# DeepLearningZ/chanamq

Hardware: AMD Instinct MI355X
Metric: msgs/sec (whole node) + p50 publish→deliver latency, 1 KB payload, 1/2/4/8 GPUs (higher is better)
Workload: dtype uint8 (AMQP wire bytes; no floating-point compute)

## Files before the change

chanamq_amd/engine/dataplane.py:

```python

import ctypes
import time
from collections import defaultdict

import os

import numpy as np

from .. import ops
from ..protocol import constants as C
from .control import ControlError, ControlState
from .layout import (CONN_OUT, CONSUMED_REC, EGRESS_REF, RING_MOVE, CTRL_REC, CTRL_DGET, CTRL_TXBUF, INVALID, MF_HAS_TS,
                     MF_HOSTPUB, MF_PERSIST,
                     MF_ONEQ, MF_REDELIVERED, MF_RESTORE,
                     PERSIST_HDR, RDESC, SEG_IN, SEG_OUT, SS_CTRL, US_ACKED, US_PENDING, US_REQUEUE, USLOT,
                     chan_hash, direct_key, exch_hash, fnv1a64, topic_pattern_row, topic_word_offsets)

ONES64 = np.uint64((1 << 64) - 1)


def parse_persist(raw):
    raw = np.frombuffer(raw, np.uint8) if isinstance(raw, (bytes, bytearray)) else raw
    hdrs, data_of, off = [], {}, 0
    while off + PERSIST_HDR.itemsize <= len(raw):
# ... 848 lines not shown
            self.eng.launch(p)
            self._pending = self._xprev = p
            return (p, len(segs), t0, self.eng.egress_slot(p))
        p = self.eng.submit(segs, int(payload_ptr), int(payload_len), now, self.step_no, now, self.worker)
        self.step_no += 1
        if self.world > 1:
            self._pending = p
            cnt = self.eng.send_counts(p)
            if cnt[-1]:
                raise RuntimeError("cross-rank send buffers overflowed (xfer_desc_max / xfer_bytes)")
            self._send_counts = cnt[:-1]
            if self.exchanger is not None:
                recv = self.exchanger.exchange(self._send_counts, self.xfer_send_desc(), self.xfer_send_pay(),
                                               self.xfer_recv_desc(), self.xfer_recv_pay())
                if self.lag:
                    self.set_import(recv)
                else:
                    self.submit_b(recv)
        return (p, len(segs), t0, self.eng.egress_slot(p))

    def prefetch(self, payload_ptr, payload_len):
        return bool(self.eng.prefetch(int(payload_ptr), int(payload_len)))

    def submit_lockstep(self, segs, payload_ptr, payload_len, now_ms=None):
        if not (self.world > 1 and self.native_xchg):
            raise RuntimeError("submit_lockstep: needs a sharded plane built with native_xchg=1")
        now = int(time.time() * 1000) if now_ms is None else int(now_ms)
        t0 = time.perf_counter()
        p = self.eng.submit(segs, int(payload_ptr), int(payload_len), now, self.step_no, now, self.worker)
        self.step_no += 1
        q = self._xprev
        if q is not None:
            rc, _ = self.eng.exchange(q, 0)
            if rc != 0:
                self.eng.drop_exchange(q)
                raise RuntimeError(f"rank {self.rank}: native exchange failed (rc {rc}: a peer did not answer)")
        self.eng.launch_b(p)
        self._xprev = p
        return (p, len(segs), t0, self.eng.egress_slot(p))

    def _exchange_parity(self, q):
        cnt = self.eng.send_counts(q)
        if cnt[-1]:
            raise RuntimeError("cross-rank send buffers overflowed (xfer_desc_max / xfer_bytes)")
        self._send_counts = cnt[:-1]
        recv = self.exchanger.exchange(self._send_counts, self._xs[q][0], self._xs[q][1],
# ... 119 lines not shown
```

csrc/kernels/dataplane.hip:

```cpp
#include "dp_state.h"
#include "dp_util.h"

DEV void apply_deltas(const DS& d, const u8* buf, u32 tid, u32 nt, DeltaRec* lrec) {
  const DeltaHead h = *(const DeltaHead*)buf;
  const DeltaRec* recs = (const DeltaRec*)(buf + sizeof(DeltaHead));
  const u32* dirty = (const u32*)(recs + h.nrec);
  const uint4* data = (const uint4*)((const u8*)dirty + ((4u * h.ndirty + 15u) & ~15u));
  for (u32 r = tid; r < h.nrec; r += nt) lrec[r] = recs[r];
  __syncthreads();
  for (u32 i = tid; i < h.nchunk; i += nt) {
    u32 lo = 0, hi = h.nrec;
    while (hi - lo > 1) {
      const u32 mid = (lo + hi) >> 1;
      if (lrec[mid].chunk0 <= i) lo = mid; else hi = mid;
    }
    const DeltaRec r = lrec[lo];
    const u32 off = (i - r.chunk0) * 16u;
    const u32 n = r.len - off < 16u ? r.len - off : 16u;
    const uint4 v = data[i];
    u8* dst = (u8*)(uintptr_t)(r.dst + off);
    const u32 w[4] = {v.x, v.y, v.z, v.w};
    if (((uintptr_t)dst & 3) == 0 && (n & 3) == 0) {
      for (u32 k = 0; k < n / 4; ++k) ((u32*)dst)[k] = w[k];
    } else {
      for (u32 k = 0; k < n; ++k) dst[k] = (u8)(w[k >> 2] >> (8 * (k & 3)));
    }
  }
  __syncthreads();
  for (u32 k = tid; k < h.ndirty; k += nt) {
    const u32 ch = dirty[k];
    if (atomicExch(&d.ch_dirty[ch], 1u) == 0) d.dirty_list[atomicAdd(d.n_dirty, 1u)] = ch;
  }
  __threadfence();
  __syncthreads();
}
__global__ __launch_bounds__(1024) void k_apply_deltas(DS d, const u8* buf) {
  __shared__ DeltaRec lrec[DELTA_REC_MAX];
  apply_deltas(d, buf, threadIdx.x, 1024, lrec);
}

__global__ __launch_bounds__(64) void k_h2d_wait(DS d) {
  const u64 sig = d.in->h2d_sig, sig2 = d.in->h2d_sig2;
  if (!sig) return;
  const u32 lim = d.in->h2d_polls ? d.in->h2d_polls : (1u << 24);
  if (threadIdx.x == 0)
    for (u32 it = 0; it < lim; ++it) {
      if (__hip_atomic_load((const i64*)sig, __ATOMIC_RELAXED, __HIP_MEMORY_SCOPE_SYSTEM) == 0 &&
          (!sig2 || __hip_atomic_load((const i64*)sig2, __ATOMIC_RELAXED, __HIP_MEMORY_SCOPE_SYSTEM) == 0))
        break;
      __builtin_amdgcn_s_sleep(4);
    }
  __syncthreads();
  __builtin_amdgcn_fence(__ATOMIC_ACQUIRE, "");
}

__global__ __launch_bounds__(1024) void k_stage(DS d) {
  __shared__ u32 lds[1024 / 64 + 1];
  __shared__ StepIn s_in;
  __shared__ DeltaRec lrec[DELTA_REC_MAX];
  const u32 tid = threadIdx.x;
  if (tid == 0) {
    s_in = *d.in_h;
    *d.in = s_in;
  }
  __syncthreads();
  if (s_in.delta_bytes) apply_deltas(d, d.delta_h, tid, 1024, lrec);
  const u32 nseg = s_in.nseg;
  {
    u32* c = (u32*)d.ctr;
    for (u32 k = tid; k < sizeof(Counters) / 4; k += 1024)
      if (k * 4 < offsetof(Counters, log_head)) c[k] = 0;
    if (tid == 0) {
      d.ctr->n_grow = 0; d.tot[TS_NMOVE] = 0; d.tot[TS_NDEFER] = 0; d.tot[TS_TTL_BUDGET] = 0;
      d.tot[TS_NDGET] = 0;
      d.tot[TS_SPILL_USED] = 0;
      d.tot[TS_HOP_N] = 0;
// ... 3480 lines not shown
```

csrc/kernels/dp_frame_scan.h:

```cpp
#pragma once
#include "dp_state.h"
#include "dp_util.h"

struct FInfo { u32 type, ch, size; bool complete, valid_hdr; };

DEV FInfo frame_at(const u8* b, u32 p, u32 L, u32 fmax) {
  FInfo f;
  f.complete = false;
  f.valid_hdr = false;
  f.type = 0; f.ch = 0; f.size = 0;
  if (p + 7 > L) return f;
  f.type = b[p];
  f.ch = be16(b + p + 1);
  f.size = be32(b + p + 3);
  bool tok = f.type == 1 || f.type == 2 || f.type == 3 || f.type == 8;
  bool sok = fmax == 0 || f.size + 8 <= fmax;
  f.valid_hdr = tok && sok;
  if (f.valid_hdr && (u64)p + 8 + f.size <= L) f.complete = (b[p + 7 + f.size] == 0xCE);
  return f;
}

DEV i32 chan_lookup(const DS& d, u32 conn, u32 ch) {
  const u32* m = d.chmap + (u64)conn * d.chmap_size;
  u32 mask = d.chmap_size - 1;
// ... 91 lines not shown
    const i32 v = d.x_hval[slot];
    if (v < 0) break;
    if (d.x_hkey[slot] == hk) { xs = v; break; }
  }
  if (xs < 0 || d.x_type[xs] != EX_DIRECT) return false;
  const u64 k = fnv1a64_dev(name, n) ^ (u64(xs) * 0x9E3779B97F4A7C15ULL);
  for (u32 j = 0; j <= d.dhash_mask; ++j) {
    const u32 s = (u32)(k + j) & d.dhash_mask;
    const i32 ex = d.d_exch[s];
    if (ex < 0) return false;
    if (ex == xs && d.d_key[s] == k && word_eq(d.kpool + d.d_kb_off[s], d.d_kb_len[s], name, n)) {
      if (d.d_q_n[s] != 1) return false;
      const u32 qq = d.d_q[d.d_q_off[s]];
      const u32 ex_owner = d.q_excl[qq];
      if (!d.q_active[qq] || d.q_owner[qq] != d.my_rank || (ex_owner && ex_owner != conn + 1)) return false;
      q = qq;
      noack = b[a + 1 + n] & 1u;
      return true;
    }
  }
  return false;
}

DEV void frame_scan_seg(const DS& d, const u32 s) {
  __shared__ uint4 fs_pool[FS_POOL / 16];
  __shared__ u32 sc[FS_NT / 64 + 1];
  __shared__ u32 sh_m, sh_over, sh_ok, sh_nf, sh_stop, sh_brk;
  __shared__ u32 sh_cmd_base, sh_frag_base, sh_ncmd;
  __shared__ u32 sh_get0, sh_gch, sh_gq, sh_gna, sh_gbase;
  __shared__ u32 sh_split;

  const u32 tid = threadIdx.x;
  const u32 conn = d.segs[s].conn;
  const u32 L = d.seg_total[s];
  const u32 seg_len = d.segs[s].len, seg_cl = L - seg_len, src = d.segs[s].src;
  const u64 ing_rel = (u64)d.in->ingress - (u64)d.work;
  const bool ing_ok = d.scan_inplace && d.world == 1 && (u64)d.in->ingress > (u64)d.work && ing_rel + src + L + 64 < (1ull << 32) &&
                      d.tot[TS_WORK_USED] <= d.work_cap;
  const bool inplace = ing_ok && seg_cl == 0 && L > 0;
  const u32 wbase = inplace ? (u32)(ing_rel + src) : d.seg_start[s];
  const u8* const bg = d.work + wbase;
  const u8* b = bg;
  const u32 nm16 = (L + 15) >> 4;
  const bool staged = nm16 * 16 + 32 <= FS_STAGE;
  const u32 cmax = staged ? FS_CAND_STAGED : CAND_MAX;
  u8* const pool = (u8*)fs_pool;
  uint4* const fs_stage = fs_pool;
  u32* const wend = (u32*)(pool + (staged ? FS_STAGE : 0u));
  u32* const cpos = wend + cmax;
  u16* const chain_am = (u16*)(cpos + cmax);
  u16* const chain = chain_am;
  u16* const amask = chain_am;
  int16_t* const csucc = (int16_t*)(chain_am + (staged ? FS_CAND_STAGED : (CAND_MAX > FS_AM_MAX ? CAND_MAX : FS_AM_MAX)));
  u8* const claim = (u8*)(csucc + cmax);
  const u32 fmax = d.conn_frame_max[conn];
  FS_MARK(15);
  const u8* const seg_C = d.carry + (u64)conn * d.carry_cap;
  const u8* const seg_N = (const u8*)d.in->ingress + d.segs[s].src;
  const bool fit = d.tot[TS_WORK_USED] <= d.work_cap;
  const bool fuse = fit && !inplace && L > 0 && ((L + 15) >> 4) <= FS_AM_MAX && !d.conn_paused[conn];
  const bool split = fuse && staged && ing_ok;
  if (fit && !fuse && !inplace) {
    u8* const dst = d.work + wbase;
    if (seg_cl) block_copy(dst, seg_C, seg_cl, tid, FS_NT);
    if (seg_len) block_copy(dst + seg_cl, seg_N, seg_len, tid, FS_NT);
  }
  __threadfence_block();
  __syncthreads();
  SegOut so;
  so.conn = conn; so.status = 0; so.consumed = 0; so.carry = L; so.ncmds = 0; so.err_off = 0;
  so.pad[0] = so.pad[1] = 0;

  if (d.conn_paused[conn]) {
    if (L > d.carry_cap) { so.status = SS_TOO_LARGE; so.carry = 0; }
    else block_copy(d.carry + (u64)conn * d.carry_cap, b, L, tid, FS_NT);
    if (tid == 0) {
      so.status |= SS_PAUSED;
      d.carry_len[conn] = so.carry;
      d.seg_out[s] = so;
      d.seg_cmd_base[s] = INVALID;
      d.seg_npub[s] = 0;
// ... 573 lines not shown
  }

  FS_MARK(7);
  u32 rest = L - consumed;
  if (rest > d.carry_cap) { so.status |= SS_TOO_LARGE; rest = 0; }
  else if (split) {
    u8* const cd = d.carry + (u64)conn * d.carry_cap;
    if (consumed < sp) block_copy(cd, d.work + wbase + consumed, sp - consumed, tid, FS_NT);
    const u32 from = consumed > sp ? consumed : sp;
    if (from < L) block_copy(cd + (from - consumed), seg_N + (from - seg_cl), L - from, tid, FS_NT);
  } else block_copy(d.carry + (u64)conn * d.carry_cap, bg + consumed, rest, tid, FS_NT);
  FS_MARK(8);
  if (tid == 0) {
    so.consumed = consumed;
    so.carry = rest;
    so.ncmds = run;
    d.carry_len[conn] = rest;
    if (reason == 0) d.conn_paused[conn] = 1;
    d.seg_out[s] = so;
  }
#undef CPOS
}

__global__ __launch_bounds__(FS_NT) void k_frame_scan(DS d) {
  const u32 nseg = d.in->nseg;
  for (u32 s = blockIdx.x; s < nseg; s += gridDim.x) {
    frame_scan_seg(d, s);
    __syncthreads();
  }
}

DEV void dget_to_host(const DS& d, u32 k) {
  const DGet g = d.dget[k];
  u32 cbase;
  const u32 got = reserve_sat(&d.ctr->ctrl_bytes, g.raw_len, (u32)d.ctrl_cap, &cbase);
  const u32 ri = atomicAdd(&d.ctr->n_ctrl, 1u);
  CtrlRec rec;
  rec.conn = g.conn;
  if (got == g.raw_len) {
    for (u32 k = 0; k < g.raw_len; ++k) d.ctrl[cbase + k] = d.work[g.raw_off + k];
    rec.off = cbase; rec.len = g.raw_len; rec.seg = CTRL_DGET | g.seg;
  } else {
    rec.off = INVALID; rec.len = 506; rec.seg = 0;
  }
  if (ri < d.seg_max * 2) d.ctrl_rec[ri] = rec;
}
```

csrc/kernels/dp_state.h:

```cpp
#pragma once
#include "dp_common.h"

#define CAND_MAX 8192
#define ID_WORKERS 64
#define ID_SLOT_BITS 18
#define DEC_SEG_LDS 4096
#define SORT_TILE 1024
#define TOPIC_K 256
#define TOPIC_WORDS 8
#define LAT_BINS 32
#define WORLD_MAX 16
#define INGRESS_SLOTS 3
#define EGRESS_SLOTS 4
#define RUNS_PER_Q 64
#define SPILL_LAG 6

enum : u32 {
  XC_SEND_N = 0, XC_SEND_B = WORLD_MAX, XC_RECV_N = 2 * WORLD_MAX, XC_RECV_B = 3 * WORLD_MAX,
  XC_OVF = 4 * WORLD_MAX, XC_RECV_AN = 4 * WORLD_MAX + 4, XC_RECV_AB = 5 * WORLD_MAX + 4,
  XC_LINK_N = 6 * WORLD_MAX + 4, XC_LINK_B = 7 * WORLD_MAX + 4, XC_ACK_N = 8 * WORLD_MAX + 4,
  XC_RACK_N = 9 * WORLD_MAX + 4, XC_WORDS = 10 * WORLD_MAX + 8
};

enum : u32 {
// ... 4 lines not shown
  TS_DELIV_BYTES = 6,
  TS_CONN_BYTES = 7,
  TS_FREE_TOP = 8,
  TS_WORK_USED = 15,
  TS_RANGE_LO = 20, TS_RANGE_HI = 21,
  TS_PAIR_BASE = 22, TS_PAIR_N = 23,
  TS_NIMPORT = 24, TS_IMPORT_BASE = 25,
  TS_PERSIST = 26,
  TS_NRUNS = 27,
  TS_REQ_TICKET = 28,
  TS_RS_TICKET = 29,
  TS_NMOVE = 30,
  TS_NDEFER = 31,
  TS_RP_TICKET = 14,
  TS_XSCAN = 32,
  TS_TTL_BUDGET = 64,
  TS_NRACK = 65,
  TS_PK_TICKET = 66,
  TS_POST_TICKET = 67,
  TS_NCADEF = 68,
  TS_NDGET = 69,
  TS_SPILL_USED = 70,
  TS_DQ_TICKET = 71,
  TS_HOP_N = 72
};

#define DGET_MAX 4096
struct DGet { u32 conn, chslot, q, noack, raw_off, raw_len, seg, pad; };

struct AckRec { u32 tq; u32 pad; u64 xid; };

enum : u32 {
  SF_NODISPATCH = 1
};

struct DS {
  u32 c_max, chpc, q_max, x_max, cons_max, seg_max;
  u32 carry_cap, cmd_max, frag_max, pub_max, ack_max, pair_max, deliv_max, msg_max;
  u32 ucap_mask, deliver_cap, chmap_size, xhash_mask, dhash_mask, tb_max, tb_pad, req_max;
  u32 q_bits, ch_bits, hash_wildcard, frame_max_global;
  u64 log_bytes, log_block, n_log_blocks, work_cap, ingress_cap, egress_cap, ctrl_cap, ring_pool;

  StepIn* in;
  const SegIn* segs;
  const StepIn* in_h;
  const SegIn* segs_h;
  const u8* delta_h;
// ... 227 lines not shown
```

csrc/kernels/engine.hip:

```cpp
#include <pybind11/pybind11.h>
#include <pybind11/numpy.h>
#include <pybind11/stl.h>

#include <chrono>
#include <algorithm>
#include <functional>
#include <map>
#include <memory>
#include <mutex>
#include <condition_variable>
#include <thread>
#include <type_traits>
#include <stdexcept>
#include <string>
#include <vector>

#include <hsa/amd_hsa_signal.h>
#include <hsa/hsa.h>
#include <hsa/hsa_ext_amd.h>
#include <rocprofiler-sdk-roctx/roctx.h>

#include "dataplane.hip"
#include "delta_stage.h"
#include "xchg_host.h"
// ... 178 lines not shown
      const u64 need = d_.work_cap + d_.xfer_bytes + 56ull * d_.pair_max + 4096;
      if (d_.persist_bytes < need) d_.persist_bytes = need;
      if (d_.persist_max < d_.pair_max) d_.persist_max = d_.pair_max;
    }
    if (d_.import_bytes + 8192 > (4ull << 30))
      throw std::runtime_error("import buffer must stay below 4 GiB (u32 offsets): lower ingress_cap / egress_cap");
    d_.ctrl_cap = get("ctrl_cap", 4ull << 20);
    d_.ring_pool = get("ring_pool", 1ull << 26);
    u32 fan_max = (u32)get("fan_max", 1u << 20);
    u32 dq_max = (u32)get("dq_max", 1u << 20);
    hopx_max_ = (u32)get("hopx_max", 1u << 16);
    const u32 hopx_max = hopx_max_;
    u64 kpool = get("kpool", 16ull << 20);
    u32 nch = d_.c_max * d_.chpc;
    d_.rank_bits = d_.world > 1 ? 1 : 0;
    d_.q_bits = bits_for(d_.q_max);
    if (d_.q_bits + d_.rank_bits > 32) throw std::runtime_error("q_max too large for sharded pair keys");
    d_.ch_bits = bits_for(nch);
    graph_enabled_ = get("graph", 1) != 0;
    copy_mode_ = (int)get("copy_engine", 0);
    sdma_ = copy_mode_ == 1;
    copy_wgs_ = (u32)get("copy_wgs", 16);
    sdma_pref_ = cfg.contains("sdma_engine") ? cfg["sdma_engine"].cast<int>() : -1;
    h2d_split_cfg_ = get("h2d_split", 0) != 0;
    h2d_split_min_ = get("h2d_split_min", 4u << 20);
    wait_ms_ = (u32)get("wait_timeout_ms", 10000);
    sdma_split_ = cfg.contains("sdma_split") ? std::max(1, std::min(2, cfg["sdma_split"].cast<int>())) : 1;

    auto dev = [&](const char* name, size_t bytes) { return alloc(name, bytes, false); };
    auto hst = [&](const char* name, size_t bytes) { return alloc(name, bytes, true); };
    d_.ctr = (Counters*)dev("ctr", sizeof(Counters));
    egress_alloc_ = d_.egress_cap + d_.work_cap + (u64)nch * 21 + 4096 + 16ull * d_.deliv_max;
    {
      const u64 wb = (d_.work_cap + 4096 + 255) & ~255ull, ib = (d_.ingress_cap + 64 + 255) & ~255ull;
      u8* base = (u8*)dev("work_all", 2 * wb + INGRESS_SLOTS * ib);
      d_.work = (u8*)view("work", base, d_.work_cap + 4096);
      work_p1_ = (u8*)view("work_p1", base + wb, d_.work_cap + 4096);
      for (int k = 0; k < INGRESS_SLOTS; ++k)
        ing_[k].buf = (u8*)view(("ingress_s" + std::to_string(k)).c_str(), base + 2 * wb + k * ib, d_.ingress_cap + 64);
    }
    npar_ = (d_.world == 1 && get("overlap", 1) == 0 && get("parities", 2) >= 3) ? 3 : 2;
    for (int e = 0; e < EGRESS_SLOTS; ++e) {
      std::string sfx = std::to_string(e);
      EgressSlot& es = eg_[e];
      es.dev = (u8*)dev(("egress" + sfx).c_str(), egress_alloc_);
      if (copy_mode_ == 2) {
        es.host = (u8*)mapped(&es.host_dev, "egress_host" + sfx, egress_alloc_);
// ... 536 lines not shown
    o["spill_bytes"] = d_.spill_bytes;
    o["hop_qmax"] = (u32)HOP_QMAX; o["hop_xslots"] = (u32)HOP_XSLOTS; o["hopx_max"] = hopx_max_;
    o["ingress_cap"] = d_.ingress_cap; o["egress_cap"] = d_.egress_cap; o["ring_pool"] = d_.ring_pool;
    o["work_cap"] = d_.work_cap; o["total_bytes"] = total_bytes_; o["req_max"] = d_.req_max;
    o["carry_budget"] = carry_budget_;
    o["exchange_lag"] = lag_ ? 1 : 0;
    o["native_xchg"] = native_x_ ? 1 : 0;
    o["rccl_standin"] = (rccl_ && cmqx::RcclLib::get().standin) ? 1 : 0;
    o["links"] = links_ ? 1 : 0;
    o["import_bytes"] = d_.import_bytes;
    o["world"] = d_.world; o["rank"] = d_.my_rank; o["import_max"] = d_.import_max; o["pub_cap"] = d_.pub_cap;
    o["copy_engine"] = copy_mode_ == 3 ? "hsa-sdma" : copy_mode_ == 2 ? "kernel" : (sdma_ ? "nocu" : "blit");
    o["copy_wgs"] = copy_wgs_;
    o["egress_gate"] = gated_ ? 1 : 0;
    o["egress_ref_back"] = ref_back_;
    o["egress_ref_min"] = ref_min_;
    o["egress_slots"] = EGRESS_SLOTS;
    o["parities"] = npar_;
    auto engine_no = [](bool used, u32 mask) { return used && mask ? __builtin_ctz(mask) : -1; };
    o["sdma_engine"] = engine_no(copy_mode_ == 3, (u32)sdma_engine_);
    o["sdma_engine2"] = engine_no(true, (u32)sdma_engine2_);
    o["h2d_hsa_engine"] = engine_no(h2d_hsa_, (u32)ing_engine_);
    o["h2d_hsa_engine2"] = engine_no(h2d_hsa_, (u32)ing_engine2_);
    o["persist"] = d_.persist; o["persist_max"] = d_.persist_max; o["persist_bytes"] = d_.persist_bytes;
    o["restore_max"] = restore_max_;
    o["xfer_desc_max"] = d_.xfer_desc_max; o["xfer_bytes"] = d_.xfer_bytes; o["world_max"] = WORLD_MAX;
    o["sizeof"] = py::dict(py::arg("StepIn") = sizeof(StepIn), py::arg("SegIn") = sizeof(SegIn),
                           py::arg("SegOut") = sizeof(SegOut), py::arg("Counters") = sizeof(Counters),
                           py::arg("CtrlRec") = sizeof(CtrlRec), py::arg("ConnOut") = sizeof(ConnOut),
                           py::arg("MsgEnt") = sizeof(MsgEnt), py::arg("Desc") = sizeof(Desc),
                           py::arg("USlot") = sizeof(USlot), py::arg("Deliv") = sizeof(Deliv),
                           py::arg("Pub") = sizeof(Pub), py::arg("Cmd") = sizeof(Cmd),
                           py::arg("RDesc") = sizeof(RDesc));
    return o;
  }

 private:
  int device_ = 0;
  u32 n_cu_ = 256;
  DS d_;
  bool graph_enabled_ = true;
  bool overlap_ = false;
  int npar_ = 2;
  bool lag_ = false, native_x_ = false, links_ = false;
  u32 restore_max_ = 0;
  u64 carry_budget_ = 0;
  int copy_mode_ = 0;
  bool sdma_ = true;
  u32 copy_wgs_ = 16;
  u32 hopx_max_ = 1u << 16;
  int sdma_pref_ = -1, sdma_split_ = 1;
  bool gated_ = false;
  bool h2d_hsa_ = false;
  bool h2d_split_cfg_ = false;
  u64 h2d_split_min_ = 4u << 20;
  u32 wait_ms_ = 10000;
  int ref_back_ = -1;
  u32 ref_min_ = 256;
 public:
  u32 dcap_bytes_ = 0;
 private:
  std::map<std::string, Buf> bufs_;
  u64 total_bytes_ = 0;
  u64 egress_alloc_ = 0;
  u32 ntiles_max_ = 0;
  u64* scan_status_ = nullptr;
  u32* scan_ctl_ = nullptr;
  u64* scan_status_ing_ = nullptr;
  u32* scan_ctl_ing_ = nullptr;
  u32 scan_smax_ = 0;
  u8* work_p1_ = nullptr;
  std::vector<std::function<void(DS&)>> par1_;
  template <class T>
  void dup(T* DS::*m, const char* name, size_t bytes) {
    T* p1 = (T*)alloc((std::string(name) + "_p1").c_str(), bytes, false);
    par1_.push_back([m, p1](DS& io) { io.*m = p1; });
  }
  u64 get_cap_ = 0;
// ... 216 lines not shown
  void ingress_copy(u64 step, int is, u64 ptr, u64 len, hipStream_t ps) {
    IngressSlot& ig = ing_[is];
    const u64 src = h2d_hsa_ ? ingress_src(ptr) : 0;
    if (src) {
      if (step >= INGRESS_SLOTS && ig.read_issued && hipEventQuery(ig.ev_read) != hipSuccess)
        HIPCHECK(hipEventSynchronize(ig.ev_read));
      if (ig.hsa) bounded_wait(ig.sig, -1, "ingress H2D");
      if (ig.split) bounded_wait(ig.sig2, -1, "ingress H2D");
      const bool split = ing_engine2_ && len >= h2d_split_min_ && len > 8192;
      const u64 h1 = split ? ((len / 2 + 4095) & ~u64(4095)) : len;
      hsa_signal_store_relaxed(ig.sig, 1);
      if (hsa_amd_memory_async_copy_on_engine(ig.buf, gpu_agent_, (const void*)src, cpu_agent_, h1, 0,
                                              nullptr, ig.sig, ing_engine_, true) != HSA_STATUS_SUCCESS)
        throw std::runtime_error("hsa_amd_memory_async_copy_on_engine (ingress) failed");
      if (split) {
        hsa_signal_store_relaxed(ig.sig2, 1);
        if (hsa_amd_memory_async_copy_on_engine(ig.buf + h1, gpu_agent_, (const void*)(src + h1), cpu_agent_,
                                                len - h1, 0, nullptr, ig.sig2, ing_engine2_,
                                                true) != HSA_STATUS_SUCCESS)
          throw std::runtime_error("hsa_amd_memory_async_copy_on_engine (ingress, second half) failed");
      }
      ig.hsa = true;
      ig.split = split;
      return;
    }
    if (step >= INGRESS_SLOTS && ig.read_issued && hipEventQuery(ig.ev_read) != hipSuccess)
      HIPCHECK(hipStreamWaitEvent(ps, ig.ev_read, 0));
    HIPCHECK(hipMemcpyAsync((void*)ig.buf, (const void*)ptr, len,
                            sdma_ ? hipMemcpyDeviceToDeviceNoCU : hipMemcpyHostToDevice, ps));
    ig.hsa = false;
    ig.split = false;
  }

  void stage_gets(const GetReq* r, u32 n) {
    if (pend_gets_.size() + n > GET_STEP_MAX) throw std::runtime_error("stage_gets: more than GET_STEP_MAX per step");
    for (u32 i = 0; i < n; ++i) {
      if (r[i].q >= d_.q_max || r[i].chslot >= d_.c_max * d_.chpc) throw std::runtime_error("stage_gets: bad queue / channel");
      pend_gets_.push_back(r[i]);
    }
  }
  py::list get_out_py(int p) {
    const StepSlot& sp = par(p);
    const GetOut* go = sp.io.get_out_hh;
    py::list l;
    for (u32 i = 0; i < sp.nget; ++i) l.append(py::make_tuple(go[i].status, go[i].msg_count));
    return l;
  }

// ... 146 lines not shown
        throw std::runtime_error("ingress copy of step " + std::to_string(sp.launch_seq) +
                                 " did not complete before its step ran (HSA SDMA copy lost)");
      }
    }
    const u64 n = sp.io.ctr_host_h->egress_bytes;
    eg_hist_[eg_hist_i_++ & 3] = n;
    eg_stats_[3] += n;
  }

  void sync() {
    HIPCHECK(hipStreamSynchronize(s_h2d_));
    if (s_h2d_alt_) HIPCHECK(hipStreamSynchronize(s_h2d_alt_));
    HIPCHECK(hipStreamSynchronize(s_pre_));
    HIPCHECK(hipStreamSynchronize(s_ing_));
    HIPCHECK(hipStreamSynchronize(s_comp_));
    HIPCHECK(hipStreamSynchronize(s_d2h_));
  }

  py::dict host_times(bool reset) {
    static const char* names[9] = {"submit", "submit_sdma_wait", "submit_graph_launch", "wait_results",
                                   "egress_copy", "egress_wait", "exchange", "exchange_counts", "exchange_thread"};
    py::dict o;
    for (int i = 0; i < 9; ++i) { o[names[i]] = ht_[i]; if (reset) ht_[i] = 0; }
    return o;
  }

  py::dict counters(int p) {
    const Counters& c = *par(p).io.ctr_host_h;
    py::dict o;
#define F(x) o[#x] = c.x
    F(n_cmds); F(n_frags); F(n_pubs); F(n_acks); F(n_ctrl); F(ctrl_bytes); F(n_pairs); F(n_deliv);
    F(egress_bytes); F(n_returns); F(n_confirm_frames); F(n_freed); F(n_requeue); F(n_unroutable);
    F(n_dropped_nomem); F(n_expired); F(n_routed_msgs); F(n_unknown_exchange); F(n_ring_full);
    F(n_acked); F(log_head); F(log_tail); F(msg_free_top); F(n_live_msgs);
    F(n_persist); F(n_consumed); F(persist_used); F(n_persist_overflow);
    F(live_bytes); F(n_grow); F(n_dget); F(spill_moved); F(n_ref); F(gath_off); F(ref_bytes);
#undef F
    std::vector<u32> lat(c.lat_hist, c.lat_hist + LAT_BINS);
    o["lat_hist"] = lat;
    return o;
  }

  u64 egress_copy(int p) {
    HostTimer ht(&ht_[4]);
    Range rg("chanamq.K5.egress_d2h");
    StepSlot& sp = par(p);
// ... 177 lines not shown
    if (sdma_pref_ >= 0 && (mask >> sdma_pref_) & 1u) pick = (u32)sdma_pref_;
    else if ((mask >> 1) & 1u) pick = 1;
    else while (!((mask >> pick) & 1u)) ++pick;
    sdma_engine_ = (hsa_amd_sdma_engine_id_t)(1u << pick);
    sdma_engine2_ = (hsa_amd_sdma_engine_id_t)0;
    if (sdma_split_ > 1)
      for (u32 c : {2u, 3u, 0u})
        if (c != pick && ((mask >> c) & 1u)) { sdma_engine2_ = (hsa_amd_sdma_engine_id_t)(1u << c); break; }
    tail_engine_ = sdma_engine_;
    for (u32 c : {2u, 3u, 0u})
      if (c != pick && ((mask >> c) & 1u) && (1u << c) != (u32)sdma_engine2_) {
        tail_engine_ = (hsa_amd_sdma_engine_id_t)(1u << c);
        break;
      }
    ing_engine_ = (hsa_amd_sdma_engine_id_t)0;
    for (u32 c : {0u, 3u, 2u, 1u})
      if (((mask >> c) & 1u) && (1u << c) != (u32)sdma_engine_ && (1u << c) != (u32)sdma_engine2_ &&
          (1u << c) != (u32)tail_engine_) {
        ing_engine_ = (hsa_amd_sdma_engine_id_t)(1u << c);
        break;
      }
    if (!ing_engine_) ing_engine_ = tail_engine_;
    ing_engine2_ = (hsa_amd_sdma_engine_id_t)0;
    if (h2d_split_cfg_)
      for (u32 c : {3u, 2u})
        if (((mask >> c) & 1u) && (1u << c) != (u32)ing_engine_ && (1u << c) != (u32)sdma_engine_ &&
            (1u << c) != (u32)sdma_engine2_ && (1u << c) != (u32)tail_engine_) {
          ing_engine2_ = (hsa_amd_sdma_engine_id_t)(1u << c);
          break;
        }
    for (EgressSlot& es : eg_)
      if (hsa_signal_create(0, 0, nullptr, &es.sdma_sig) != HSA_STATUS_SUCCESS ||
          hsa_signal_create(0, 0, nullptr, &es.tail_sig) != HSA_STATUS_SUCCESS ||
          hsa_signal_create(0, 0, nullptr, &es.gate_sig) != HSA_STATUS_SUCCESS)
        throw std::runtime_error("hsa_signal_create failed");
  }

  void drain_egress() {
    for (int e = 0; e < EGRESS_SLOTS; ++e) {
      sdma_wait(e);
      if (eg_[e].d2h_issued) HIPCHECK(hipEventSynchronize(eg_[e].ev_d2h));
    }
  }

  std::vector<u32> send_counts(int p) {
    StepSlot& sp = par(p);
    if (!sp.counts_ready) throw std::runtime_error("send_counts: no phase-A step in flight for this parity");
    sp.counts_ready = false;
    HIPCHECK(hipEventSynchronize(sp.ev_a));
    const u32* x = sp.io.xchg_h;
    std::vector<u32> o;
    for (u32 r = 0; r < d_.world; ++r) o.push_back(x[r]);
    for (u32 r = 0; r < d_.world; ++r) o.push_back(x[WORLD_MAX + r]);
// ... 758 lines not shown
    const u32 ntiles = ceil_div(nmax, SORT_TILE);
    const u32 digit = bits > 8 && bits <= 11 ? bits : 8;
    u32 src = 0;
    for (u32 shift = 0; shift < bits; shift += digit) {
      with_key_bits(digit, [&](auto b) {
        constexpr u32 B = decltype(b)::value;
        hipLaunchKernelGGL(k_rs_hist<B>, capped(ntiles, 256), dim3(RsNt<B>::v), 0, s, keys[src], n, shift, d_.hist,
                           d_.hist_scan, &d.tot[TS_RS_TICKET], ntiles);
        hipLaunchKernelGGL(k_rs_scatter<B>, capped(ntiles, 256), dim3(256), 0, s, keys[src], vals[src], keys[src ^ 1],
                           vals[src ^ 1], n, shift, d_.hist_scan, ntiles);
      });
      src ^= 1;
    }
    return src;
  }

  static dim3 blocks(u64 n, u32 per) { return dim3(n ? ceil_div(n, per) : 1); }
  static dim3 wave_blocks(u64 n) { u64 b = n ? ceil_div(n, 4) : 1; return dim3(b > 8192 ? 8192 : (u32)b); }
  static dim3 capped(u64 b, u32 cap) { return dim3(b == 0 ? 1u : (b > cap ? cap : (u32)b)); }

  void launch_ingest(hipStream_t s, const DS& d) {
    Range rg("chanamq.K1-K4.ingest");
    hipLaunchKernelGGL(k_stage, dim3(1), dim3(1024), 0, s, d);
    if (h2d_hsa_) hipLaunchKernelGGL(k_h2d_wait, dim3(16), dim3(64), 0, s, d);
    hipLaunchKernelGGL(k_frame_scan, capped(d.seg_max, n_cu_), dim3(FS_NT), 0, s, d);
    if (d.rank_scan)
      launch_scan(s, d, {{d.cmd_is_pub, d.cmd_pub_rank}, {d.cmd_is_ack, d.cmd_ack_rank}}, &d.ctr->n_cmds,
                  d.cmd_max, TS_CMD_PUBS, nullptr, true);
    hipLaunchKernelGGL(k_decode, blocks(d.cmd_max, 256), dim3(256), 0, s, d);
  }

  void launch_route(hipStream_t s, const DS& d, u32 nmax, bool imports = false) {
    Range rg("chanamq.K6-K13.route_store");
    const u64 ngroups = ceil_div(nmax ? nmax : 1, 16);
    if (imports) hipLaunchKernelGGL(k_import_route, capped(ngroups, n_cu_), dim3(1024), 0, s, d);
    else hipLaunchKernelGGL(k_route, capped(ngroups, 2 * n_cu_), dim3(1024), 0, s, d);
    const ScanArgs a = scan_args({{d.pub_nq, d.pub_pair_off}, {d.pub_slot, d.pub_slot_off},
                                  {d.pub_routed, d.pub_routed_rank}, {d.pub_ret_sz, d.pub_ret_off}},
                                 &d.tot[TS_RANGE_HI], d.pub_cap, TS_ROUTE, &d.tot[TS_RANGE_LO]);
    hipLaunchKernelGGL(k_scan_route, dim3(ceil_div(d.pub_cap ? d.pub_cap : 1, SCAN_TILE)), dim3(1024), 0, s, a, d.tot,
                       scan_status_, scan_ctl_, scan_smax_, d);
    hipLaunchKernelGGL(k_route_store, wave_blocks(nmax), dim3(256), 0, s, d, imports ? 0u : 1u);
  }

  void launch_pack(hipStream_t s, const DS& d) {
    Range rg("chanamq.X1.pack");
    hipLaunchKernelGGL(k_pack_scan, blocks(d.pub_max, PK_TILE), dim3(1024), 0, s, d, d.pk_agg, &d.tot[TS_PK_TICKET]);
    hipLaunchKernelGGL(k_pack, wave_blocks(d.pub_max), dim3(256), 0, s, d);
// ... 135 lines not shown
           })
      .def("get_out", &Engine::get_out_py)
      .def("send_counts", &Engine::send_counts)
      .def("submit_b", &Engine::submit_b, py::arg("parity"), py::arg("recv"), py::arg("stream") = 0)
      .def("set_xfer_buffers", &Engine::set_xfer_buffers)
      .def("set_xfer_parity", &Engine::set_xfer_parity)
      .def("set_import", &Engine::set_import, py::arg("recv"), py::arg("stream") = 0)
      .def("restore", &Engine::restore, py::arg("desc"), py::arg("payload"), py::arg("now_ms"))
      .def("spill", &Engine::spill, py::arg("lim"), py::arg("hot"), py::call_guard<py::gil_scoped_release>())
      .def("cold_pick", &Engine::cold_pick, py::arg("hot"), py::arg("lim"), py::arg("max_n"), py::arg("max_bytes"))
      .def("cold_commit", &Engine::cold_commit)
      .def("cold_scan", &Engine::cold_scan, py::arg("window"), py::arg("max_n"))
      .def("cold_in", &Engine::cold_in)
      .def("side_cold_pick", &Engine::side_cold_pick, py::arg("hot"), py::arg("lim"), py::arg("min_used"),
           py::arg("max_n"), py::arg("max_bytes"))
      .def("side_cold_commit", &Engine::side_cold_commit)
      .def("side_cold_scan", &Engine::side_cold_scan, py::arg("window"), py::arg("max_n"))
      .def("side_cold_in", &Engine::side_cold_in)
      .def("side_cold_live", &Engine::side_cold_live)
      .def("side_wait", &Engine::side_wait, py::arg("timeout_s"))
      .def("side_pending", &Engine::side_pending)
      .def("basic_get", &Engine::basic_get, py::arg("q"), py::arg("chslot"), py::arg("noack"), py::arg("now_ms"))
      .def("wait_results", &Engine::wait_results)
      .def("egress_copy", &Engine::egress_copy)
      .def("egress_wait", &Engine::egress_wait)
      .def("egress_slot", &Engine::egress_slot)
      .def("set_egress_ref", &Engine::set_egress_ref)
      .def("set_deliver_cap_bytes", [](Engine& e, u32 n) { e.dcap_bytes_ = n; })
      .def("egress_wait_slot", &Engine::egress_wait_slot)
      .def("egress_done_slot", &Engine::egress_done_slot)
      .def("step_done", &Engine::step_done)
      .def("sync", &Engine::sync)
      .def("c_api", &Engine::c_api)
      .def("xchg_setup", &Engine::xchg_setup, py::arg("kind"), py::arg("arg"), py::arg("members"),
           py::arg("timeout_ms") = 10000, py::arg("failover") = false, py::arg("counts_shm") = "",
           py::arg("async_x") = false,
           py::call_guard<py::gil_scoped_release>())
      .def_static("xchg_unique_id", &Engine::xchg_unique_id)
      .def("exchange", [](Engine& e, int q, u32 flags) {
             u32 orf = 0;
             int rc;
             {
               py::gil_scoped_release nogil;
               rc = e.exchange(q, flags, &orf);
             }
             return py::make_tuple(rc, orf);
// ... 19 lines not shown
```

Baseline: 48.87 million.

## Fold H2D wait into frame scan and enable split H2D copies by default

Merges the separate H2D-completion wait kernel into k_frame_scan when the grid is large enough. Block 0 polls the host signals and publishes a step marker, and the other blocks spin on that marker after prefetching their segment headers. This removes one kernel launch per step and overlaps the header loads with the copy wait. It also turns on h2d_split by default, widens the search for a second SDMA engine (including engine 0 or the tail engine), and adds H2D counters plus profiling scripts. The risk is that the split engines now contend with egress SDMA, and blocks spin-waiting inside the scan kernel tie up CUs.

Measured after the change: 49.40 million (median of 6 runs). 1.01x the previous value.

```diff
diff --git a/chanamq_amd/engine/dataplane.py b/chanamq_amd/engine/dataplane.py
--- a/chanamq_amd/engine/dataplane.py
+++ b/chanamq_amd/engine/dataplane.py
@@ -894,6 +894,9 @@
     def prefetch(self, payload_ptr, payload_len):
         return bool(self.eng.prefetch(int(payload_ptr), int(payload_len)))
 
+    def h2d_stats(self):
+        return dict(self.eng.h2d_stats())
+
     def submit_lockstep(self, segs, payload_ptr, payload_len, now_ms=None):
         if not (self.world > 1 and self.native_xchg):
             raise RuntimeError("submit_lockstep: needs a sharded plane built with native_xchg=1")
diff --git a/csrc/kernels/dataplane.hip b/csrc/kernels/dataplane.hip
--- a/csrc/kernels/dataplane.hip
+++ b/csrc/kernels/dataplane.hip
@@ -37,21 +37,6 @@
 __global__ __launch_bounds__(1024) void k_apply_deltas(DS d, const u8* buf) {
   __shared__ DeltaRec lrec[DELTA_REC_MAX];
   apply_deltas(d, buf, threadIdx.x, 1024, lrec);
-}
-
-__global__ __launch_bounds__(64) void k_h2d_wait(DS d) {
-  const u64 sig = d.in->h2d_sig, sig2 = d.in->h2d_sig2;
-  if (!sig) return;
-  const u32 lim = d.in->h2d_polls ? d.in->h2d_polls : (1u << 24);
-  if (threadIdx.x == 0)
-    for (u32 it = 0; it < lim; ++it) {
-      if (__hip_atomic_load((const i64*)sig, __ATOMIC_RELAXED, __HIP_MEMORY_SCOPE_SYSTEM) == 0 &&
-          (!sig2 || __hip_atomic_load((const i64*)sig2, __ATOMIC_RELAXED, __HIP_MEMORY_SCOPE_SYSTEM) == 0))
-        break;
-      __builtin_amdgcn_s_sleep(4);
-    }
-  __syncthreads();
-  __builtin_amdgcn_fence(__ATOMIC_ACQUIRE, "");
 }
 
 __global__ __launch_bounds__(1024) void k_stage(DS d) {
diff --git a/csrc/kernels/dp_frame_scan.h b/csrc/kernels/dp_frame_scan.h
--- a/csrc/kernels/dp_frame_scan.h
+++ b/csrc/kernels/dp_frame_scan.h
@@ -137,7 +137,18 @@
   return false;
 }
 
-DEV void frame_scan_seg(const DS& d, const u32 s) {
+struct FsHead { u32 conn, L, seg_len, src, fmax; };
+DEV FsHead fs_head(const DS& d, const u32 s) {
+  FsHead h;
+  h.conn = d.segs[s].conn;
+  h.L = d.seg_total[s];
+  h.seg_len = d.segs[s].len;
+  h.src = d.segs[s].src;
+  h.fmax = d.conn_frame_max[h.conn];
+  return h;
+}
+
+DEV void frame_scan_seg(const DS& d, const u32 s, const FsHead hd) {
   __shared__ uint4 fs_pool[FS_POOL / 16];
   __shared__ u32 sc[FS_NT / 64 + 1];
   __shared__ u32 sh_m, sh_over, sh_ok, sh_nf, sh_stop, sh_brk;
@@ -146,9 +157,9 @@
   __shared__ u32 sh_split;
 
   const u32 tid = threadIdx.x;
-  const u32 conn = d.segs[s].conn;
-  const u32 L = d.seg_total[s];
-  const u32 seg_len = d.segs[s].len, seg_cl = L - seg_len, src = d.segs[s].src;
+  const u32 conn = hd.conn;
+  const u32 L = hd.L;
+  const u32 seg_len = hd.seg_len, seg_cl = L - seg_len, src = hd.src;
   const u64 ing_rel = (u64)d.in->ingress - (u64)d.work;
   const bool ing_ok = d.scan_inplace && d.world == 1 && (u64)d.in->ingress > (u64)d.work && ing_rel + src + L + 64 < (1ull << 32) &&
                       d.tot[TS_WORK_USED] <= d.work_cap;
@@ -168,10 +179,10 @@
   u16* const amask = chain_am;
   int16_t* const csucc = (int16_t*)(chain_am + (staged ? FS_CAND_STAGED : (CAND_MAX > FS_AM_MAX ? CAND_MAX : FS_AM_MAX)));
   u8* const claim = (u8*)(csucc + cmax);
-  const u32 fmax = d.conn_frame_max[conn];
+  const u32 fmax = hd.fmax;
   FS_MARK(15);
   const u8* const seg_C = d.carry + (u64)conn * d.carry_cap;
-  const u8* const seg_N = (const u8*)d.in->ingress + d.segs[s].src;
+  const u8* const seg_N = (const u8*)d.in->ingress + src;
   const bool fit = d.tot[TS_WORK_USED] <= d.work_cap;
   const bool fuse = fit && !inplace && L > 0 && ((L + 15) >> 4) <= FS_AM_MAX && !d.conn_paused[conn];
   const bool split = fuse && staged && ing_ok;
@@ -791,10 +802,42 @@
 #undef CPOS
 }
 
-__global__ __launch_bounds__(FS_NT) void k_frame_scan(DS d) {
+DEV void h2d_wait(const DS& d) {
+  const u64 sig = d.in->h2d_sig, sig2 = d.in->h2d_sig2;
+  if (!sig) return;
+  const u32 lim = d.in->h2d_polls ? d.in->h2d_polls : (1u << 24);
+  const u32 seen = (u32)d.in->step + 1u;
+  if (threadIdx.x < 64) {
+    if (threadIdx.x != 0) {
+    } else if (blockIdx.x == 0) {
+      for (u32 it = 0; it < lim; ++it) {
+        if (__hip_atomic_load((const i64*)sig, __ATOMIC_RELAXED, __HIP_MEMORY_SCOPE_SYSTEM) == 0 &&
+            (!sig2 || __hip_atomic_load((const i64*)sig2, __ATOMIC_RELAXED, __HIP_MEMORY_SCOPE_SYSTEM) == 0))
+          break;
+        __builtin_amdgcn_s_sleep(4);
+      }
+      __hip_atomic_store(&d.tot[TS_H2D_SEEN], seen, __ATOMIC_RELAXED, __HIP_MEMORY_SCOPE_AGENT);
+    } else {
+      for (u32 it = 0; it < lim; ++it) {
+        if (__hip_atomic_load(&d.tot[TS_H2D_SEEN], __ATOMIC_RELAXED, __HIP_MEMORY_SCOPE_AGENT) == seen) break;
+        __builtin_amdgcn_s_sleep(4);
+      }
+    }
+    __builtin_amdgcn_fence(__ATOMIC_ACQUIRE, "");
+  }
+  __syncthreads();
+}
+
+__global__ __launch_bounds__(64) void k_h2d_wait(DS d) { h2d_wait(d); }
+
+__global__ __launch_bounds__(FS_NT) void k_frame_scan(DS d, u32 wait) {
   const u32 nseg = d.in->nseg;
+  if (!wait && blockIdx.x >= nseg) return;
+  FsHead hd{};
+  if (blockIdx.x < nseg) hd = fs_head(d, blockIdx.x);
+  if (wait) h2d_wait(d);
   for (u32 s = blockIdx.x; s < nseg; s += gridDim.x) {
-    frame_scan_seg(d, s);
+    frame_scan_seg(d, s, s == blockIdx.x ? hd : fs_head(d, s));
     __syncthreads();
   }
 }
diff --git a/csrc/kernels/dp_state.h b/csrc/kernels/dp_state.h
--- a/csrc/kernels/dp_state.h
+++ b/csrc/kernels/dp_state.h
@@ -50,7 +50,8 @@
   TS_NDGET = 69,
   TS_SPILL_USED = 70,
   TS_DQ_TICKET = 71,
-  TS_HOP_N = 72
+  TS_HOP_N = 72,
+  TS_H2D_SEEN = 73
 };
 
 #define DGET_MAX 4096
diff --git a/csrc/kernels/engine.hip b/csrc/kernels/engine.hip
--- a/csrc/kernels/engine.hip
+++ b/csrc/kernels/engine.hip
@@ -224,7 +224,7 @@
     sdma_ = copy_mode_ == 1;
     copy_wgs_ = (u32)get("copy_wgs", 16);
     sdma_pref_ = cfg.contains("sdma_engine") ? cfg["sdma_engine"].cast<int>() : -1;
-    h2d_split_cfg_ = get("h2d_split", 0) != 0;
+    h2d_split_cfg_ = get("h2d_split", 1) != 0;
     h2d_split_min_ = get("h2d_split_min", 4u << 20);
     wait_ms_ = (u32)get("wait_timeout_ms", 10000);
     sdma_split_ = cfg.contains("sdma_split") ? std::max(1, std::min(2, cfg["sdma_split"].cast<int>())) : 1;
@@ -807,6 +807,8 @@
     o["sdma_engine2"] = engine_no(true, (u32)sdma_engine2_);
     o["h2d_hsa_engine"] = engine_no(h2d_hsa_, (u32)ing_engine_);
     o["h2d_hsa_engine2"] = engine_no(h2d_hsa_, (u32)ing_engine2_);
+    o["egress_tail_engine"] = engine_no(copy_mode_ == 3, (u32)tail_engine_);
+    o["h2d_split_min"] = h2d_split_min_;
     o["persist"] = d_.persist; o["persist_max"] = d_.persist_max; o["persist_bytes"] = d_.persist_bytes;
     o["restore_max"] = restore_max_;
     o["xfer_desc_max"] = d_.xfer_desc_max; o["xfer_bytes"] = d_.xfer_bytes; o["world_max"] = WORLD_MAX;
@@ -837,8 +839,9 @@
   int sdma_pref_ = -1, sdma_split_ = 1;
   bool gated_ = false;
   bool h2d_hsa_ = false;
-  bool h2d_split_cfg_ = false;
+  bool h2d_split_cfg_ = true;
   u64 h2d_split_min_ = 4u << 20;
+  u64 h2d_n_[3] = {0, 0, 0};
   u32 wait_ms_ = 10000;
   int ref_back_ = -1;
   u32 ref_min_ = 256;
@@ -1101,8 +1104,10 @@
       }
       ig.hsa = true;
       ig.split = split;
+      ++h2d_n_[split ? 0 : 1];
       return;
     }
+    ++h2d_n_[2];
     if (step >= INGRESS_SLOTS && ig.read_issued && hipEventQuery(ig.ev_read) != hipSuccess)
       HIPCHECK(hipStreamWaitEvent(ps, ig.ev_read, 0));
     HIPCHECK(hipMemcpyAsync((void*)ig.buf, (const void*)ptr, len,
@@ -1295,6 +1300,14 @@
                                    "egress_copy", "egress_wait", "exchange", "exchange_counts", "exchange_thread"};
     py::dict o;
     for (int i = 0; i < 9; ++i) { o[names[i]] = ht_[i]; if (reset) ht_[i] = 0; }
+    return o;
+  }
+
+  py::dict h2d_stats() const {
+    py::dict o;
+    o["split"] = h2d_n_[0]; o["unsplit"] = h2d_n_[1]; o["runtime"] = h2d_n_[2];
+    o["engine"] = h2d_hsa_ && ing_engine_ ? __builtin_ctz((u32)ing_engine_) : -1;
+    o["engine2"] = h2d_hsa_ && ing_engine2_ ? __builtin_ctz((u32)ing_engine2_) : -1;
     return o;
   }
 
@@ -1518,13 +1531,17 @@
       }
     if (!ing_engine_) ing_engine_ = tail_engine_;
     ing_engine2_ = (hsa_amd_sdma_engine_id_t)0;
-    if (h2d_split_cfg_)
-      for (u32 c : {3u, 2u})
+    if (h2d_split_cfg_) {
+      for (u32 c : {3u, 2u, 0u})
         if (((mask >> c) & 1u) && (1u << c) != (u32)ing_engine_ && (1u << c) != (u32)sdma_engine_ &&
             (1u << c) != (u32)sdma_engine2_ && (1u << c) != (u32)tail_engine_) {
           ing_engine2_ = (hsa_amd_sdma_engine_id_t)(1u << c);
           break;
         }
+      if (!ing_engine2_ && tail_engine_ != sdma_engine_ && tail_engine_ != sdma_engine2_ && tail_engine_ != ing_engine_ &&
+          __builtin_ctz((u32)tail_engine_) < 4)
+        ing_engine2_ = tail_engine_;
+    }
     for (EgressSlot& es : eg_)
       if (hsa_signal_create(0, 0, nullptr, &es.sdma_sig) != HSA_STATUS_SUCCESS ||
           hsa_signal_create(0, 0, nullptr, &es.tail_sig) != HSA_STATUS_SUCCESS ||
@@ -2329,8 +2346,10 @@
   void launch_ingest(hipStream_t s, const DS& d) {
     Range rg("chanamq.K1-K4.ingest");
     hipLaunchKernelGGL(k_stage, dim3(1), dim3(1024), 0, s, d);
-    if (h2d_hsa_) hipLaunchKernelGGL(k_h2d_wait, dim3(16), dim3(64), 0, s, d);
-    hipLaunchKernelGGL(k_frame_scan, capped(d.seg_max, n_cu_), dim3(FS_NT), 0, s, d);
+    const dim3 fs_grid = capped(d.seg_max, n_cu_);
+    const bool fold = h2d_hsa_ && fs_grid.x >= 16;
+    if (h2d_hsa_ && !fold) hipLaunchKernelGGL(k_h2d_wait, dim3(16), dim3(64), 0, s, d);
+    hipLaunchKernelGGL(k_frame_scan, fs_grid, dim3(FS_NT), 0, s, d, fold ? 1u : 0u);
     if (d.rank_scan)
       launch_scan(s, d, {{d.cmd_is_pub, d.cmd_pub_rank}, {d.cmd_is_ack, d.cmd_ack_rank}}, &d.ctr->n_cmds,
                   d.cmd_max, TS_CMD_PUBS, nullptr, true);
@@ -2512,6 +2531,7 @@
       .def("side_pending", &Engine::side_pending)
       .def("basic_get", &Engine::basic_get, py::arg("q"), py::arg("chslot"), py::arg("noack"), py::arg("now_ms"))
       .def("wait_results", &Engine::wait_results)
+      .def("h2d_stats", &Engine::h2d_stats)
       .def("egress_copy", &Engine::egress_copy)
       .def("egress_wait", &Engine::egress_wait)
       .def("egress_slot", &Engine::egress_slot)
diff --git a/profiles/link_rate/link_counters.py b/profiles/link_rate/link_counters.py
--- /dev/null
+++ b/profiles/link_rate/link_counters.py
@@ -0,0 +1,44 @@
+#!/usr/bin/env python3
+import json
+import os
+import sys
+
+sys.path.insert(0, os.getcwd())
+
+import bench
+from chanamq_amd.engine.dataplane import GpuDataPlane
+
+
+def main(steps=12):
+    P, Q, chunk, blocks = 256, 16, 49152, 8
+    cfg = dict(c_max=max(1024, P + Q + 1), chpc=4, q_max=Q + 64, cons_max=1024, seg_max=1024, cmd_max=1 << 17,
+               deliv_max=1 << 16, msg_max=1 << 22, ucap=4096, deliver_cap=8192, ingress_cap=32 << 20,
+               egress_cap=128 << 20, log_bytes=16 << 30, ring_pool=Q * (1 << 20) + Q + 1024, tb_max=64,
+               fan_max=1 << 20, carry_cap=256 << 10, graph=1, copy_engine=3, sdma_engine=-1, sdma_split=1,
+               egress_gate=1, overlap=0, parities=2, h2d_alt=0, h2d_hsa=1, egress_ref=0)
+    dp = GpuDataPlane(device=0, worker=0, **cfg)
+    pool, segs, offs, blens, *_ = bench.build_workload(dp, 0, P, Q, 1024, chunk, blocks, cons_base=P)
+    base = pool.ctypes.data
+    pending = []
+    for i in range(steps):
+        b = i % blocks
+        pending.append(dp.submit_raw(segs[b], base + offs[b], blens[b]))
+        if len(pending) > 1:
+            t = pending.pop(0)
+            dp.wait(t)
+            if i + 1 < steps:
+                nb = (i + 1) % blocks
+                dp.prefetch(base + offs[nb], blens[nb])
+            dp.finish(t, collect=False, waited=True)
+    for t in pending:
+        dp.finish(t, collect=False)
+    info = dp.info
+    print(json.dumps({
+        "steps": steps, "payload_bytes": sorted(set(int(x) for x in blens)),
+        "h2d_split_min": info["h2d_split_min"],
+        "engines": {k: info[k] for k in ("sdma_engine", "egress_tail_engine", "h2d_hsa_engine", "h2d_hsa_engine2")},
+        "h2d_stats": dp.h2d_stats()}, indent=1))
+
+
+if __name__ == "__main__":
+    main(int(sys.argv[1]) if len(sys.argv) > 1 else 12)
diff --git a/profiles/link_rate/trace_model.py b/profiles/link_rate/trace_model.py
--- /dev/null
+++ b/profiles/link_rate/trace_model.py
@@ -0,0 +1,71 @@
+#!/usr/bin/env python3
+import csv
+import glob
+import json
+import statistics
+import sys
+
+
+def rows(d, pat):
+    f = glob.glob(f"{d}/**/*{pat}*.csv", recursive=True)
+    if not f:
+        raise SystemExit(f"no *{pat}*.csv under {d}")
+    with open(f[0], newline="") as fh:
+        return list(csv.DictReader(fh))
+
+
+def main(d, timed=50):
+    ks = sorted(((r["Kernel_Name"].split("(")[0].replace("void ", ""), int(r["Start_Timestamp"]), int(r["End_Timestamp"]))
+                 for r in rows(d, "kernel_trace")), key=lambda k: k[1])
+    cp = sorted(((int(r["Start_Timestamp"]), int(r["End_Timestamp"]), r.get("Direction", "")) for r in rows(d, "memory_copy_trace")),
+                key=lambda c: c[0])
+    pay = [c for c in cp if "HOST_TO_DEVICE" in c[2].upper().replace("2", "_TO_") and c[1] - c[0] > 50_000]
+    groups = []
+    for c in pay:
+        if groups and c[0] - groups[-1][0][0] < 30_000:
+            groups[-1].append(c)
+        else:
+            groups.append([c])
+    copies = [(min(c[0] for c in g), max(c[1] for c in g), len(g)) for g in groups]
+    steps = []
+    for n, s, e in ks:
+        if n.startswith("k_stage"):
+            steps.append({})
+        if steps:
+            steps[-1].setdefault(n, (s, e))
+            steps[-1]["_sum"] = steps[-1].get("_sum", 0) + (e - s)
+            steps[-1]["_n"] = steps[-1].get("_n", 0) + 1
+    steps = [s for s in steps if any(n.startswith("k_post") for n in s)]
+    head_of = lambda s: next(v for k, v in s.items() if k.startswith("k_frame_scan"))
+    paired = []
+    for s in steps:
+        mine = [c for c in copies if c[1] <= head_of(s)[1]]
+        if mine and (not paired or mine[-1] is not paired[-1][1]):
+            paired.append((s, mine[-1]))
+    steps, copies = [p[0] for p in paired], [p[1] for p in paired]
+    n = len(steps)
+    post = [next(v for k, v in s.items() if k.startswith("k_post")) for s in steps]
+    head = [head_of(s) for s in steps]
+    lo, hi = max(2, n - timed), n - 2
+    us = lambda x: round(statistics.median(x) / 1e3, 1)
+    out = {
+        "steps": hi - lo,
+        "halves_per_payload": statistics.median(c[2] for c in copies[lo:hi]),
+        "H_us": us([copies[i][1] - copies[i][0] for i in range(lo, hi)]),
+        "C_us": us([post[i][1] - max(copies[i][1], head[i][0]) for i in range(lo, hi)]),
+        "delta_us": us([copies[i + 1][0] - post[i - 1][1] for i in range(lo, hi - 1)]),
+        "copy_idle_us": us([copies[i + 1][0] - copies[i][1] for i in range(lo, hi - 1)]),
+        "P_us": us([copies[i + 1][0] - copies[i][0] for i in range(lo, hi - 1)]),
+        "kernel_sum_us": us([steps[i]["_sum"] for i in range(lo, hi)]),
+        "kernels_per_step": statistics.median(steps[i]["_n"] for i in range(lo, hi)),
+        "copy_end_to_post_end_us": us([post[i][1] - copies[i][1] for i in range(lo, hi)]),
+        "per_kernel_us": {k: us([steps[i][k][1] - steps[i][k][0] for i in range(lo, hi) if k in steps[i]])
+                          for k in steps[hi - 1] if not k.startswith("_")},
+    }
+    H, C, dl = out["H_us"], out["C_us"], out["delta_us"]
+    out["model_P_us"] = round(max(H, (H + C + dl) / 2), 1)
+    print(json.dumps(out, indent=1))
+
+
+if __name__ == "__main__":
+    main(sys.argv[1], int(sys.argv[2]) if len(sys.argv) > 2 else 50)
```
